# C0ldstudy/PointSecGuard

Measured on AMD Instinct MI355X. Metric: attacked rooms/sec (4096 pts, 40 PGD iters), higher is better.
Workload: dtype f32; 1 GPU; NB non-targeted PGD (eps=0.05, alpha=2/255, 40 iters) on PointNet++ SSG sem_seg, batch=8 rooms x 4096 pts x 9 ch per GPU (BASELINE configs[1]); steps_coalesced_per_launch_max=8, device_batch_rooms=64, launches_in_flight_per_gpu=3, weights=tests/golden/pn2_weights.npz (fitted fixture)

## Files before the change

pointsecguard_amd/csrc/psg_pn2.hip:

```cpp
#include <algorithm>
#include <cstdlib>
#include <cstring>
#include <vector>

#include "psg_common.h"
#include "psg_pn2_kernels.cuh"
#include "psg_chain.cuh"
#include "psg_pn2_geomgrad.cuh"

using namespace psg;

namespace {

constexpr int MAXL = PSG_PN2_MSG_NUM_LAYERS;
constexpr int NCLS = PSG_PN2_NUM_CLASSES;
const int kS[4] = {1024, 256, 64, 16};

static inline int diag_build_bits()
{
#ifdef PSG_DIAG_BUILD
    static const int bits = psg::env_int("PSG_DIAG", 0);
    return bits;
#else
    return 0;
// ... 91 lines not shown
    return arch_split(A, lvl) || (l0 && A.id == PSG_PN2_ARCH_SSG && lvl == 0);
}

bool arch_fp_split(const ArchDesc &A, int lvl)
{
    static const bool on = psg::env_int("PSG_PN2_FPSPLIT", 1) != 0, wave1 = psg::env_int("PSG_FP1_WAVE", 0) != 0;
    return on && lvl <= 2 && !(lvl == 0 && wave1);
}

bool arch_pack(const ArchDesc &A)
{
    static const bool on = psg::env_int("PSG_PN2_PACK", 1) != 0;
    return on && A.id == PSG_PN2_ARCH_SSG;
}

constexpr int kPackBwdBuilt = 1 << 0;
int pack_bwd_levels()
{
    static const int levels = [] {
        const char *v = psg::env_str("PSG_PN2_PACK_BWD");
        if (!v || !*v) return kPackBwdBuilt;
        if (*v == 'L' || *v == 'l') {
            int mask = 1 << 8;
            for (const char *c = v + 1; *c; ++c)
                if (*c >= '0' && *c <= '3') mask |= 1 << (*c - '0');
            return mask;
        }
        return atoi(v) != 0 ? kPackBwdBuilt : 0;
    }();
    return levels;
}
// ... 172 lines not shown
    EvScope prof(&ws->prof, tag, 0.0, st);
    hipLaunchKernelGGL(kern, grid, dim3(threads), lds, st, args);
    PSG_LAUNCH_CHECK_AT(site);
    return PSG_OK;
}

inline int layer_blocks(int k8, int mb) { return std::max(k8, mb * 4); }
inline int gsa_stride(const ArchDesc &A, int lvl)
{
    if (arch_split(A, lvl)) return A.cout[A.sc[lvl][0].l0];
    return lvl == 0 ? 12 : A.C[lvl];
}

#define PSG_CFG_KEY(P, NW, KS, MT) ((P) * 10000 + (NW) * 1000 + (KS) * 10 + (MT))

bool sa_pack_bwd_level(const psg_pn2_model *m, const psg_pn2_ws *ws, int lvl)
{
    const int levels = pack_bwd_levels();
    if (!ws->pk_cnt[lvl] || !((levels >> lvl) & 1)) return false;
    if (levels >> 8) return true;
    return lvl == 0 && !m->split_fwd[0] && !m->split[0] && m->split[1];
}

int run_sa_fwd(psg_pn2_model *m, psg_pn2_ws *ws, int lvl, int sc, int fwd, const float *x0, hipStream_t st)
{
    const ArchDesc &A = *m->arch;
    const ScaleDesc &d = A.sc[lvl][sc];
    const int B = ws->B, S = kS[lvl], Np = ws->Nl[lvl], D = A.C[lvl], KS = d.K, P = d.P, NW = d.NW;
    const PackedLayer *L = &m->L[d.l0];
    const size_t prob = (size_t)fwd * B;
    SaFwdArgs a;
    a.diag = diag_build_bits();
    a.xyz = lvl == 0 ? x0 : ws->xyz[lvl] + prob * Np * 3;
    a.xyz_stride = lvl == 0 ? 9 : 3;
    a.feat = lvl == 0 ? x0 : ws->act[lvl - 1];
    a.new_xyz = ws->xyz[lvl + 1] + prob * S * 3;
// ... 15 lines not shown
        return PSG_ERR_STATE;
    }
    const dim3 grid(S / (P / KS), B);
    const int tag = TAG_SA_FWD + lvl;
    a.pk_desc = nullptr; a.pk_tab_off = 0;
    const int blk = P * 8 + PSG_LDS_PAD;
    const bool pkm = sa_pack_bwd_level(m, ws, lvl);
    if (ws->pk_cnt[lvl] && KS == 32 && d.maxt_f == 1 && split == (lvl >= 1) && a.nb3 * (P / 32) == 2 * NW &&
        blocks * blk + 2 * P <= (P - 1) * a.C3 && (P * a.C3) % blk == 0) {
        a.pk_desc = ws->pk_desc[lvl] + prob * grid.x;
        a.pk_tab_off = blocks * blk;
        const int pblocks = P * a.C3 / blk;
        if (pkm) {
            switch (PSG_CFG_KEY(P, NW, KS, split ? 1 : 0)) {
            case PSG_CFG_KEY(128, 4, 32, 0): return launch_lds(ws, tag, PSG_SITE "#packed", (sa_fwd_packed_kernel<128, 4, false, true>), grid, 4 * 64, pblocks, blk, a, st);
            }
            set_error("run_sa_fwd level %d: PSG_PN2_PACK_BWD names a level without a packed-key forward kernel (P=%d NW=%d)", lvl, P, NW);
            return PSG_ERR_STATE;
        }
        switch (PSG_CFG_KEY(P, NW, KS, split ? 1 : 0)) {
        case PSG_CFG_KEY(128, 4, 32, 0): return launch_lds(ws, tag, PSG_SITE "#packed", (sa_fwd_packed_kernel<128, 4, false>), grid, 4 * 64, pblocks, blk, a, st);
        case PSG_CFG_KEY(64, 4, 32, 1): return launch_lds(ws, tag, PSG_SITE "#packed", (sa_fwd_packed_kernel<64, 4, true>), grid, 4 * 64, pblocks, blk, a, st);
        case PSG_CFG_KEY(32, 4, 32, 1): return launch_lds(ws, tag, PSG_SITE "#packed", (sa_fwd_packed_kernel<32, 4, true>), grid, 4 * 64, pblocks, blk, a, st);
        case PSG_CFG_KEY(32, 8, 32, 1): return launch_lds(ws, tag, PSG_SITE "#packed", (sa_fwd_packed_kernel<32, 8, true>), grid, 8 * 64, pblocks, blk, a, st);
        }
        a.pk_desc = nullptr; a.pk_tab_off = 0;
    }
    if (pkm) {
        set_error("run_sa_fwd level %d: the packed backward (PSG_PN2_PACK_BWD) needs the packed forward, which this configuration does not run", lvl);
        return PSG_ERR_STATE;
// ... 73 lines not shown
        a.nninv_off = ws->inv_off[3] + prob * (kS[3] + 1);
        a.nninv_ent = ws->inv_ent[3] + prob * ws->Nl[3] * 3;
        a.dint = ws->dint[3];
        a.n_fine = ws->Nl[3];
    }
    a.arg = ws->arg[lvl][sc];
    a.gidx = ws->gidx[lvl][sc] + prob * S * KS;
    a.l3t = bwd_layer(L[2], ws->mask[d.l0 + 1]);
    a.l2t = bwd_layer(L[1], ws->mask[d.l0]);
    a.l1t = bwd_layer(L[0], nullptr);
    a.D = D; a.Np = Np; a.S = S; a.C3 = C3;
    a.c_lo = c_lo; a.c_hi = c_hi;
    static const bool l1t_colour = psg::env_int("PSG_PN2_L1T_COLOUR", 1) != 0;
    a.w1c = nullptr; a.C1 = L[0].cout; a.w1c_off = 0;
    if (l1t_colour && a.cg_out == 4 && !a.split && P == 32 * NW && (a.C1 == 16 || a.C1 == 32)) a.w1c = m->w1feat[sc];
    static const bool poolt_sparse = psg::env_int("PSG_PN2_POOLT_SPARSE", 1) != 0;
    const int C2 = L[2].cin, NT = NW * 64;
    const int spv = poolt_sparse && L[2].wr && KS == 32 && P <= 64 && (P / KS) * C3 <= NT && C3 % 64 == 0 && !a.w1c &&
                    (C2 == 64 || C2 == 128 || C2 == 256) ? C2 / 64 : 0;
    const int l3_blocks = spv ? a.l3t.mb * 4 : layer_blocks(a.l3t.k8, a.l3t.mb);
    const int main_blocks = std::max(std::max(l3_blocks, layer_blocks(a.l2t.k8, a.l2t.mb)),
                                     a.split ? 0 : layer_blocks(a.l1t.k8, a.l1t.mb)) + PSG_LDS_SPARE;
    a.dsrc_blk = main_blocks;
    const int blk_floats = P * 8 + PSG_LDS_PAD;
    a.w1c_off = round_up((P / KS) * C3, 4);
    a.pos_off = a.w1c_off + (a.w1c ? round_up(3 * a.C1, 4) : 0);
    a.sp_off = round_up(a.pos_off + P, 4);
    a.w3r = spv ? L[2].wr : nullptr;
    const bool packed = sa_pack_bwd_level(m, ws, lvl);
    if (packed) {
        if (spv || a.split || !a.dout || a.nninv_off || a.ginv_off || ((a.ld | a.c_off) & 3) || (C3 & 7) ||
            PSG_CFG_KEY(P, NW, KS, d.maxt_b) != PSG_CFG_KEY(128, 4, 32, 1)) {
            set_error("run_sa_bwd level %d: PSG_PN2_PACK_BWD names a level without a packed backward kernel in this configuration", lvl);
            return PSG_ERR_STATE;
        }
    }
    const int staged = spv ? a.sp_off + 2 * NT + NW * 32 + P + 1 : a.pos_off + P + (packed ? P : 0);
    const int blocks = main_blocks + ceil_div(staged, blk_floats);
    if (std::max(std::max(a.l3t.mb, a.l2t.mb), a.split ? 0 : a.l1t.mb) * (P / 32) > d.maxt_b * NW) {
        set_error("run_sa_bwd level %d scale %d: more than %d tiles per wave in a layer", lvl, sc, d.maxt_b);
        return PSG_ERR_STATE;
    }
    const dim3 grid(S / (P / KS), B);
    const int tag = TAG_SA_BWD + lvl;
    if (packed) {
        const SaBwdPackedArgs pa{a, ws->pk_desc[lvl] + prob * grid.x};
        if (a.w1c) return launch_lds(ws, tag, PSG_SITE "#colour#bwd#packed", (sa_bwd_packed_kernel<128, 4, 1, 0>), grid, 4 * 64, blocks, Lds<128>::BLK, pa, st);
        return launch_lds(ws, tag, PSG_SITE "#bwd#packed", (sa_bwd_packed_kernel<128, 4, 1, 0>), grid, 4 * 64, blocks, Lds<128>::BLK, pa, st);
    }
#define PSG_SA_BWD_CASE(P_, NW_, KS_, MT_) \
    case PSG_CFG_KEY(P_, NW_, KS_, MT_): \
        if (a.w1c) return launch_lds(ws, tag, PSG_SITE "#colour", (sa_bwd_kernel<P_, NW_, MT_, KS_>), grid, NW_ * 64, blocks, Lds<P_>::BLK, a, st); \
        return launch_lds(ws, tag, PSG_SITE, (sa_bwd_kernel<P_, NW_, MT_, KS_>), grid, NW_ * 64, blocks, Lds<P_>::BLK, a, st)
    if (spv) {
        switch (PSG_CFG_KEY(P, NW, KS, d.maxt_b) * 8 + spv) {
        case PSG_CFG_KEY(64, 4, 32, 2) * 8 + 1: return launch_lds(ws, tag, PSG_SITE, (sa_bwd_sparse_kernel<64, 4, 2, 1>), grid, 4 * 64, blocks, Lds<64>::BLK, a, st);
        case PSG_CFG_KEY(32, 4, 32, 2) * 8 + 2: return launch_lds(ws, tag, PSG_SITE, (sa_bwd_sparse_kernel<32, 4, 2, 2>), grid, 4 * 64, blocks, Lds<32>::BLK, a, st);
        case PSG_CFG_KEY(32, 8, 32, 2) * 8 + 4: return launch_lds(ws, tag, PSG_SITE, (sa_bwd_sparse_kernel<32, 8, 2, 4>), grid, 8 * 64, blocks, Lds<32>::BLK, a, st);
        }
        set_error("run_sa_bwd: no sparse kernel for P=%d NW=%d MAXT=%d C2=%d", P, NW, d.maxt_b, C2);
        return PSG_ERR_STATE;
// ... 1304 lines not shown
```

pointsecguard_amd/csrc/psg_pn2_kernels.cuh:

```cuda
#pragma once
#include "psg_mlp.cuh"

#ifdef PSG_DIAG_BUILD
#define PSG_DIAGBIT(a, bit) ((a).diag & (bit))
#else
#define PSG_DIAGBIT(a, bit) 0
#endif

namespace psg {

struct SaFwdArgs {
    const float *xyz;
    const float *feat;
    const float *new_xyz;
    const int32_t *gidx;
    float *out;
    uint8_t *arg;
    FwdLayer l1, l2;
    const float4 *w3;
    const float *b3;
    int k8_3, nb3;
    int xyz_stride, D, Np, S, C3;
    int ld_out, c_out;
    const float *tfeat;
// ... 607 lines not shown
        const float4 z = *(const float4 *)(buf0 + L::off(c, j));
        const float4 w0 = *(const float4 *)(t + 4 * q), w1 = *(const float4 *)(t + KH + 4 * q), w2 = *(const float4 *)(t + 2 * KH + 4 * q);
        g0 = fmaf(z.x, w0.x, g0); g0 = fmaf(z.y, w0.y, g0); g0 = fmaf(z.z, w0.z, g0); g0 = fmaf(z.w, w0.w, g0);
        g1 = fmaf(z.x, w1.x, g1); g1 = fmaf(z.y, w1.y, g1); g1 = fmaf(z.z, w1.z, g1); g1 = fmaf(z.w, w1.w, g1);
        g2 = fmaf(z.x, w2.x, g2); g2 = fmaf(z.y, w2.y, g2); g2 = fmaf(z.z, w2.z, g2); g2 = fmaf(z.w, w2.w, g2);
    }
    const float o0 = __shfl_xor(g0, 32), o1 = __shfl_xor(g1, 32), o2 = __shfl_xor(g2, 32);
    if (h == 0 && pj >= 0) *(float4 *)(orow + (size_t)pj * 4) = make_float4(g0 + o0, g1 + o1, g2 + o2, 0.0f);
}

template <int SPV> struct SpVec;
template <> struct SpVec<1> { using T = float; };
template <> struct SpVec<2> { using T = float2; };
template <> struct SpVec<4> { using T = float4; };

template <int P, int NW, int MAXT, int SPV>
__device__ __forceinline__ void sa_pool_t_sparse(const SaBwdArgs &a, float *__restrict__ buf0, float *__restrict__ dsrc, int key,
                                                 size_t wg)
{
    using L = Lds<P>;
    using VT = typename SpVec<SPV>::T;
    constexpr int KS = 32, C2 = 64 * SPV, NT = NW * 64, PB = P / 32, U = 16;
    static_assert(P <= 64, "one scan lane per row");
    const int tid = threadIdx.x, lane = tid & 63, wave = tid >> 6;
    int2 *items = (int2 *)(dsrc + a.sp_off);
    int *tab = (int *)(items + NT);
    int *rs = tab + NW * KS;
    unsigned long long same = ~0ull;
#pragma unroll
    for (int bit = 0; bit < 6; ++bit) {
        const unsigned long long bb = __ballot((key >> bit) & 1);
        same &= ((key >> bit) & 1) ? bb : ~bb;
    }
    const int rank = __popcll(same & ((1ull << lane) - 1ull));
    if (key < KS && rank == 0) tab[wave * KS + key] = __popcll(same);
    __syncthreads();
    if (wave == 0) {
        const int cpg = a.C3 >> 6, g = lane / KS, k = lane & (KS - 1);
        int tot = 0;
        if (lane < P)
            for (int q = 0; q < cpg; ++q) tot += tab[(g * cpg + q) * KS + k];
        int inc = tot;
#pragma unroll
        for (int o = 1; o < 64; o <<= 1) {
            const int v = __shfl_up(inc, o);
            if (lane >= o) inc += v;
        }
        int run = inc - tot;
        if (lane < P) {
            rs[lane] = run;
            for (int q = 0; q < cpg; ++q) {
                int *t = tab + (g * cpg + q) * KS + k;
                const int c = *t;
                *t = run;
                run += c;
            }
        }
        if (lane == 63) rs[P] = inc;
    }
    __syncthreads();
    if (key < KS) {
        const int g = tid / a.C3, c = tid - g * a.C3;
        items[tab[wave * KS + key] + rank] = make_int2(((g * KS + key) << 16) | c, __float_as_int(dsrc[tid]));
    }
    const int ntask = (C2 / 32) * PB;
    unsigned msk[MAXT];
#pragma unroll
    for (int i = 0; i < MAXT; ++i) {
        const int task = wave + i * NW;
        msk[i] = 0xFFFFu;
        if (task < ntask && a.l3t.mask) msk[i] = a.l3t.mask[(wg * ntask + task) * 64 + lane];
    }
    __syncthreads();
    const int T = __builtin_amdgcn_readfirstlane(rs[P]);
    const int lo = wave * T / NW, hi = (wave + 1) * T / NW;
    const int rsl = lane < P ? rs[lane] : 0x7fffffff;
    const int r_lo = __popcll(__ballot(rsl < lo));
    const int r_hi = wave == NW - 1 ? P : __popcll(__ballot(rsl < hi));
    const int e_lo = __builtin_amdgcn_readfirstlane(rs[r_lo]), e_hi = __builtin_amdgcn_readfirstlane(rs[r_hi]);
    const float *wr = a.w3r + lane * SPV;
    float acc[SPV];
#pragma unroll
    for (int e = 0; e < SPV; ++e) acc[e] = 0.0f;
    int cur = r_lo;
    auto put = [&](int r) {
        float *o = buf0 + L::off(lane * SPV, r);
        if constexpr (SPV == 4) *(float4 *)o = make_float4(acc[0], acc[1], acc[2], acc[3]);
        else if constexpr (SPV == 2) *(float2 *)o = make_float2(acc[0], acc[1]);
        else *o = acc[0];
#pragma unroll
        for (int e = 0; e < SPV; ++e) acc[e] = 0.0f;
    };
    for (int w0 = e_lo; w0 < e_hi; w0 += 64) {
        const int n = min(64, e_hi - w0);
        const int2 mine = lane < n ? items[w0 + lane] : make_int2(0, 0);
        for (int q = 0; q < n; q += U) {
            VT w[U];
            int xs[U];
            float ds[U];
#pragma unroll
            for (int u = 0; u < U; ++u) {
                xs[u] = __builtin_amdgcn_readlane(mine.x, q + u);
                ds[u] = __int_as_float(__builtin_amdgcn_readlane(mine.y, q + u));
                if (q + u < n) w[u] = *(const VT *)(wr + (size_t)(xs[u] & 0xFFFF) * C2);
            }
#pragma unroll
            for (int u = 0; u < U; ++u) {
                if (q + u < n) {
                    const int row = xs[u] >> 16;
                    while (cur < row) put(cur++);
                    const float *wv = (const float *)&w[u];
#pragma unroll
                    for (int e = 0; e < SPV; ++e) acc[e] = fmaf(ds[u], wv[e], acc[e]);
                }
            }
        }
    }
    while (cur < r_hi) put(cur++);
    __syncthreads();
    const int j = lane & 31, h = lane >> 5;
#pragma unroll
    for (int i = 0; i < MAXT; ++i) {
        const int task = wave + i * NW;
        if (task < ntask) {
            const int mb = task / PB, pb = task - mb * PB;
            float *o = buf0 + (size_t)(mb * 4) * L::BLK + (pb * 32 + j) * 8 + 4 * h;
#pragma unroll
            for (int g = 0; g < 4; ++g) {
                float4 v = *(float4 *)(o + (size_t)g * L::BLK);
                v.x = __uint_as_float(__float_as_uint(v.x) & (unsigned)__builtin_amdgcn_sbfe((int)msk[i], 4 * g, 1));
                v.y = __uint_as_float(__float_as_uint(v.y) & (unsigned)__builtin_amdgcn_sbfe((int)msk[i], 4 * g + 1, 1));
                v.z = __uint_as_float(__float_as_uint(v.z) & (unsigned)__builtin_amdgcn_sbfe((int)msk[i], 4 * g + 2, 1));
                v.w = __uint_as_float(__float_as_uint(v.w) & (unsigned)__builtin_amdgcn_sbfe((int)msk[i], 4 * g + 3, 1));
                *(float4 *)(o + (size_t)g * L::BLK) = v;
            }
        }
    }
}

template <int P, int NW, int MAXT, int KS, int SPV, bool KEYED = false>
__device__ __forceinline__ void sa_bwd_body(const SaBwdArgs &a, int kbx = 0, int kb = 0, size_t kwg = 0)
{
    using L = Lds<P>;
    static_assert(KS == 32 || KS == 16, "groups of 32 or 16 samples");
    constexpr bool SPARSE = SPV > 0;
    static_assert(!SPARSE || KS == 32, "sparse max-pool transpose: groups of 32 samples");
    constexpr int G = P / KS, NT = NW * 64;
    extern __shared__ float lds[];
    float *buf0 = lds;
    const int tid = threadIdx.x;
    int bx, b;
    if constexpr (KEYED) { bx = kbx; b = kb; }
// ... 19 lines not shown
                const int pnt = t % P, blk = t / P;
                am_pre[i] = *(const uint2 *)(a.arg + ((size_t)b * a.S + s0 + pnt / KS) * a.C3 + blk * 8);
            }
        }
    }
    float *dsrc = lds + (size_t)a.dsrc_blk * L::BLK;
    if (SPARSE && tid < NW * KS) ((int *)(dsrc + a.sp_off) + 2 * NT)[tid] = 0;
    int32_t *s_pos = (int32_t *)(dsrc + a.pos_off);
    if (!a.w1c && tid < P) s_pos[tid] = a.gpos_out[(size_t)b * a.S * KS + (size_t)s0 * KS + tid];
    if (a.w1c && tid < 3 * a.C1) {
        const int kh = a.C1 >> 1, hh = tid / (3 * kh), r = (tid / kh) % 3, cc = tid % kh;
        dsrc[a.w1c_off + tid] = a.w1c[(hh * kh + cc) * a.D + a.c_lo + r];
    }
    for (int t = tid; t < G * a.C3; t += NT) {
        const int g = t / a.C3, c = t - g * a.C3;
        const int cc = a.c_off + c;
        float acc = a.dout ? a.dout[((size_t)b * a.S + s0 + g) * a.ld + cc] : 0.0f;
        if (a.nninv_off) {
            const int32_t *off = a.nninv_off + (size_t)b * (a.S + 1) + s0 + g;
            const int2 *ent = a.nninv_ent + (size_t)b * 3 * a.n_fine;
            const float *drows = a.dint + (size_t)b * a.n_fine * a.ld + cc;
            const int e1 = off[1];
            int e = off[0];
            for (; e + 4 <= e1; e += 4) {
                const int2 p0 = ent[e], p1 = ent[e + 1], p2 = ent[e + 2], p3 = ent[e + 3];
                const float v0 = drows[(size_t)p0.x * a.ld], v1 = drows[(size_t)p1.x * a.ld], v2 = drows[(size_t)p2.x * a.ld],
                            v3 = drows[(size_t)p3.x * a.ld];
                acc += __int_as_float(p0.y) * v0; acc += __int_as_float(p1.y) * v1;
                acc += __int_as_float(p2.y) * v2; acc += __int_as_float(p3.y) * v3;
            }
// ... 46 lines not shown
            v0.y = (int)((am.x >> 8) & 0xFF) == k ? d0.y : 0.f;
            v0.z = (int)((am.x >> 16) & 0xFF) == k ? d0.z : 0.f;
            v0.w = (int)(am.x >> 24) == k ? d0.w : 0.f;
            v1.x = (int)(am.y & 0xFF) == k ? d1.x : 0.f;
            v1.y = (int)((am.y >> 8) & 0xFF) == k ? d1.y : 0.f;
            v1.z = (int)((am.y >> 16) & 0xFF) == k ? d1.z : 0.f;
            v1.w = (int)(am.y >> 24) == k ? d1.w : 0.f;
            float *dst = buf0 + (size_t)blk * L::BLK + pnt * 8;
            *(float4 *)dst = v0;
            *(float4 *)(dst + 4) = v1;
        }
        __syncthreads();
        if (!PSG_DIAGBIT(a, 8)) layer_bwd<P, NW, MAXT>(a.l3t, buf0, wg);
    }
    if (!PSG_DIAGBIT(a, 16)) __syncthreads();
    if (!PSG_DIAGBIT(a, 8)) layer_bwd<P, NW, MAXT>(a.l2t, buf0, wg);
    if (!PSG_DIAGBIT(a, 16)) __syncthreads();
    if constexpr (P == 32 * NW) {
        if (a.w1c) {
            float *orowc = a.gsa_out + (size_t)b * a.S * KS * 4;
            const int32_t *posc = a.gpos_out + (size_t)b * a.S * KS + (size_t)s0 * KS;
            if (a.C1 == 32) sa_l1t_colour<P, NW, 32>(a, buf0, dsrc + a.w1c_off, posc, orowc);
            else sa_l1t_colour<P, NW, 16>(a, buf0, dsrc + a.w1c_off, posc, orowc);
            return;
        }
    }
    if (!a.split) {
        if (!PSG_DIAGBIT(a, 8)) layer_bwd<P, NW, MAXT>(a.l1t, buf0, wg);
        __syncthreads();
    }
    if (PSG_DIAGBIT(a, 32)) return;
// ... 53 lines not shown
            apply_bits(c, m);
            acc[i] = c;
        }
    }
    __syncthreads();
#pragma unroll
    for (int i = 0; i < MAXT; ++i) {
        const int task = first + i * NW;
        if (task < ntask) {
            const int mb = task / nblk, pb = task - mb * nblk;
            store_tile<P>(buf, mb, pb * 32 + j, h, acc[i]);
        }
    }
}

template <int P, int NW, int MAXT, int SPV>
__global__ __launch_bounds__(NW * 64) void sa_bwd_packed_kernel(SaBwdPackedArgs pa)
{
    const SaBwdArgs &a = pa.a;
    using L = Lds<P>;
    static_assert(SPV == 0 && MAXT == 1 && P == 32 * NW, "built: the dense level, one tile per wave");
    constexpr int PB = P / 32, NT = NW * 64, KS = 32;
    extern __shared__ float lds[];
    float *buf0 = lds;
    const int tid = threadIdx.x, wave = tid >> 6;
    int bx, b;
    xcd_tile(bx, b);
    const size_t wg = (size_t)b * gridDim.x + bx;
    const int4 desc = pa.pk_desc[wg];
    const int ng = desc.x >> 16, sA = desc.x & 0xFFFF;
    if (ng == 0) return;
    int nrows = 0, rg_g = 0, rg_st = 0;
    for (int i = 0; i < ng; ++i) {
        if (tid >= nrows) { rg_g = i; rg_st = nrows; }
        nrows += sa_pack_cnt(desc, i);
    }
    if (ng == PB && (sA & (PB - 1)) == 0 && nrows == P) {
        sa_bwd_body<P, NW, MAXT, KS, 0, true>(a, sA / PB, b, wg);
        return;
    }
    const int nblk = (nrows + 31) >> 5, nact = nblk * 32;
    float *dsrc = lds + (size_t)a.dsrc_blk * L::BLK;
    int32_t *s_pos = (int32_t *)(dsrc + a.pos_off);
    int *s_row = s_pos + P;
    if (tid < P) {
        int om = -1, pj = -1;
        if (tid < nrows) {
            const int k = tid - rg_st;
            om = (rg_g << 5) | k;
            pj = a.gpos_out[(size_t)b * a.S * KS + (size_t)(sA + rg_g) * KS + k];
        }
        s_row[tid] = om;
        s_pos[tid] = pj;
    }
    if (a.w1c && tid < 3 * a.C1) {
        const int kh = a.C1 >> 1, hh = tid / (3 * kh), r = (tid / kh) % 3, cc = tid % kh;
        dsrc[a.w1c_off + tid] = a.w1c[(hh * kh + cc) * a.D + a.c_lo + r];
    }
    __syncthreads();
    {
        const float *drows = a.dout + (size_t)b * a.S * a.ld + a.c_off;
        const uint8_t *arows = a.arg + (size_t)b * a.S * a.C3;
        const int nq = nblk * (a.C3 >> 3);
        const int rcp = (65536 + nblk - 1) / nblk;
#pragma unroll
        for (int i = 0; i < 4; ++i) {
            const int q = (tid >> 5) + i * (NT / 32);
            if (q < nq) {
                const int blk = (q * rcp) >> 16, pb = q - blk * nblk, j = pb * 32 + (tid & 31);
                const int om = s_row[j];
                float4 v0 = make_float4(0.f, 0.f, 0.f, 0.f), v1 = v0;
                if (om >= 0) {
                    const int s = sA + (om >> 5), k = om & 31;
                    const uint2 am = *(const uint2 *)(arows + (size_t)s * a.C3 + blk * 8);
                    const float *dp = drows + (size_t)s * a.ld + blk * 8;
                    const float4 d0 = *(const float4 *)dp, d1 = *(const float4 *)(dp + 4);
                    v0.x = (int)(am.x & 0xFF) == k ? d0.x : 0.f;
                    v0.y = (int)((am.x >> 8) & 0xFF) == k ? d0.y : 0.f;
                    v0.z = (int)((am.x >> 16) & 0xFF) == k ? d0.z : 0.f;
                    v0.w = (int)(am.x >> 24) == k ? d0.w : 0.f;
                    v1.x = (int)(am.y & 0xFF) == k ? d1.x : 0.f;
                    v1.y = (int)((am.y >> 8) & 0xFF) == k ? d1.y : 0.f;
                    v1.z = (int)((am.y >> 16) & 0xFF) == k ? d1.z : 0.f;
                    v1.w = (int)(am.y >> 24) == k ? d1.w : 0.f;
                }
                float *dst = buf0 + (size_t)blk * L::BLK + j * 8;
                *(float4 *)dst = v0;
                *(float4 *)(dst + 4) = v1;
            }
        }
    }
    __syncthreads();
    sa_layer_bwd_packed<P, NW, MAXT>(a.l3t, buf0, nblk, wg);
    __syncthreads();
    sa_layer_bwd_packed<P, NW, MAXT>(a.l2t, buf0, nblk, wg);
    __syncthreads();
    if (a.w1c) {
        if (wave < nblk) {
            float *orowc = a.gsa_out + (size_t)b * a.S * KS * 4;
            if (a.C1 == 32) sa_l1t_colour<P, NW, 32>(a, buf0, dsrc + a.w1c_off, s_pos, orowc);
            else sa_l1t_colour<P, NW, 16>(a, buf0, dsrc + a.w1c_off, s_pos, orowc);
        }
        return;
    }
    if (!a.split) {
        sa_layer_bwd_packed<P, NW, MAXT>(a.l1t, buf0, nblk, wg);
        __syncthreads();
    }
    const int nc = a.c_hi - a.c_lo;
    const int32_t *pos = s_pos;
    float *orow = a.gsa_out + (size_t)b * a.S * KS * a.cg_out;
    if (a.cg_out == 4) {
        for (int j = tid; j < nact; j += NT) {
            const float4 v = make_float4(buf0[L::off(a.c_lo, j)], buf0[L::off(a.c_lo + 1, j)], buf0[L::off(a.c_lo + 2, j)], 0.0f);
            if (pos[j] >= 0) *(float4 *)(orow + (size_t)pos[j] * 4) = v;
        }
        return;
    }
    if (((nc | a.c_lo | a.cg_out) & 3) == 0) {
        constexpr int RG = NT / 32;
        const int ql = tid & 31, rg = tid >> 5;
        for (int j = rg; j < nact; j += RG) {
// ... 613 lines not shown
```

Measured before the change: 957.3 rooms/s.

## Extend packed-row backward to sparse-pool SA levels 1-3

Enables the packed (compacted valid-row) backward path by default for SA level 1 as well as level 0, and adds packed forward/backward kernel instantiations for the split sparse-pool configurations at levels 1-3. A new packed variant of the sparse max-pool transpose scatters gradients straight into the compacted rows, iterating over groups and applying the ReLU mask tile once at the end. The goal is to skip work on padded or duplicate neighbour rows in the deeper levels. It adds extra LDS staging for group starts, a per-group loop with more barriers, and more kernel variants.

```diff
diff --git a/pointsecguard_amd/csrc/psg_pn2.hip b/pointsecguard_amd/csrc/psg_pn2.hip
--- a/pointsecguard_amd/csrc/psg_pn2.hip
+++ b/pointsecguard_amd/csrc/psg_pn2.hip
@@ -129,7 +129,7 @@
     return on && A.id == PSG_PN2_ARCH_SSG;
 }
 
-constexpr int kPackBwdBuilt = 1 << 0;
+constexpr int kPackBwdBuilt = (1 << 0) | (1 << 1);
 int pack_bwd_levels()
 {
     static const int levels = [] {
@@ -332,12 +332,22 @@
 
 #define PSG_CFG_KEY(P, NW, KS, MT) ((P) * 10000 + (NW) * 1000 + (KS) * 10 + (MT))
 
+int sa_sparse_spv(const ScaleDesc &d, const PackedLayer *L, bool w1c)
+{
+    static const bool poolt_sparse = psg::env_int("PSG_PN2_POOLT_SPARSE", 1) != 0;
+    const int C3 = L[2].cout, C2 = L[2].cin, NT = d.NW * 64;
+    return poolt_sparse && L[2].wr && d.K == 32 && d.P <= 64 && (d.P / d.K) * C3 <= NT && C3 % 64 == 0 && !w1c &&
+           (C2 == 64 || C2 == 128 || C2 == 256) ? C2 / 64 : 0;
+}
+
 bool sa_pack_bwd_level(const psg_pn2_model *m, const psg_pn2_ws *ws, int lvl)
 {
     const int levels = pack_bwd_levels();
     if (!ws->pk_cnt[lvl] || !((levels >> lvl) & 1)) return false;
     if (levels >> 8) return true;
-    return lvl == 0 && !m->split_fwd[0] && !m->split[0] && m->split[1];
+    if (lvl == 0) return !m->split_fwd[0] && !m->split[0] && m->split[1];
+    return m->split_fwd[lvl] && m->split[lvl] && (lvl == 3 || m->split[lvl + 1]) &&
+           sa_sparse_spv(m->arch->sc[lvl][0], &m->L[m->arch->sc[lvl][0].l0], false) > 0;
 }
 
 int run_sa_fwd(psg_pn2_model *m, psg_pn2_ws *ws, int lvl, int sc, int fwd, const float *x0, hipStream_t st)
@@ -383,6 +393,9 @@
         if (pkm) {
             switch (PSG_CFG_KEY(P, NW, KS, split ? 1 : 0)) {
             case PSG_CFG_KEY(128, 4, 32, 0): return launch_lds(ws, tag, PSG_SITE "#packed", (sa_fwd_packed_kernel<128, 4, false, true>), grid, 4 * 64, pblocks, blk, a, st);
+            case PSG_CFG_KEY(64, 4, 32, 1): return launch_lds(ws, tag, PSG_SITE "#packed", (sa_fwd_packed_kernel<64, 4, true, true>), grid, 4 * 64, pblocks, blk, a, st);
+            case PSG_CFG_KEY(32, 4, 32, 1): return launch_lds(ws, tag, PSG_SITE "#packed", (sa_fwd_packed_kernel<32, 4, true, true>), grid, 4 * 64, pblocks, blk, a, st);
+            case PSG_CFG_KEY(32, 8, 32, 1): return launch_lds(ws, tag, PSG_SITE "#packed", (sa_fwd_packed_kernel<32, 8, true, true>), grid, 8 * 64, pblocks, blk, a, st);
             }
             set_error("run_sa_fwd level %d: PSG_PN2_PACK_BWD names a level without a packed-key forward kernel (P=%d NW=%d)", lvl, P, NW);
             return PSG_ERR_STATE;
@@ -486,10 +499,8 @@
     static const bool l1t_colour = psg::env_int("PSG_PN2_L1T_COLOUR", 1) != 0;
     a.w1c = nullptr; a.C1 = L[0].cout; a.w1c_off = 0;
     if (l1t_colour && a.cg_out == 4 && !a.split && P == 32 * NW && (a.C1 == 16 || a.C1 == 32)) a.w1c = m->w1feat[sc];
-    static const bool poolt_sparse = psg::env_int("PSG_PN2_POOLT_SPARSE", 1) != 0;
     const int C2 = L[2].cin, NT = NW * 64;
-    const int spv = poolt_sparse && L[2].wr && KS == 32 && P <= 64 && (P / KS) * C3 <= NT && C3 % 64 == 0 && !a.w1c &&
-                    (C2 == 64 || C2 == 128 || C2 == 256) ? C2 / 64 : 0;
+    const int spv = sa_sparse_spv(d, L, a.w1c != nullptr);
     const int l3_blocks = spv ? a.l3t.mb * 4 : layer_blocks(a.l3t.k8, a.l3t.mb);
     const int main_blocks = std::max(std::max(l3_blocks, layer_blocks(a.l2t.k8, a.l2t.mb)),
                                      a.split ? 0 : layer_blocks(a.l1t.k8, a.l1t.mb)) + PSG_LDS_SPARE;
@@ -501,13 +512,18 @@
     a.w3r = spv ? L[2].wr : nullptr;
     const bool packed = sa_pack_bwd_level(m, ws, lvl);
     if (packed) {
-        if (spv || a.split || !a.dout || a.nninv_off || a.ginv_off || ((a.ld | a.c_off) & 3) || (C3 & 7) ||
-            PSG_CFG_KEY(P, NW, KS, d.maxt_b) != PSG_CFG_KEY(128, 4, 32, 1)) {
+        const bool dense0 = !spv && !a.split && a.dout && !a.nninv_off && !a.ginv_off && !((a.ld | a.c_off) & 3) && !(C3 & 7) &&
+                            PSG_CFG_KEY(P, NW, KS, d.maxt_b) == PSG_CFG_KEY(128, 4, 32, 1);
+        const bool sparse = spv && a.split && m->split_fwd[lvl] && !a.ginv_off && (a.dout != nullptr) != (a.nninv_off != nullptr) &&
+                            (P / KS) * C3 == NT && std::max(a.l3t.mb, a.l2t.mb) * (P / 32) <= NW &&
+                            (PSG_CFG_KEY(P, NW, KS, spv) == PSG_CFG_KEY(64, 4, 32, 1) || PSG_CFG_KEY(P, NW, KS, spv) == PSG_CFG_KEY(32, 4, 32, 2) ||
+                             PSG_CFG_KEY(P, NW, KS, spv) == PSG_CFG_KEY(32, 8, 32, 4));
+        if (!dense0 && !sparse) {
             set_error("run_sa_bwd level %d: PSG_PN2_PACK_BWD names a level without a packed backward kernel in this configuration", lvl);
             return PSG_ERR_STATE;
         }
     }
-    const int staged = spv ? a.sp_off + 2 * NT + NW * 32 + P + 1 : a.pos_off + P + (packed ? P : 0);
+    const int staged = spv ? a.sp_off + 2 * NT + NW * 32 + P + 1 + (packed ? SA_PACK_GCAP + 1 : 0) : a.pos_off + P + (packed ? P : 0);
     const int blocks = main_blocks + ceil_div(staged, blk_floats);
     if (std::max(std::max(a.l3t.mb, a.l2t.mb), a.split ? 0 : a.l1t.mb) * (P / 32) > d.maxt_b * NW) {
         set_error("run_sa_bwd level %d scale %d: more than %d tiles per wave in a layer", lvl, sc, d.maxt_b);
@@ -517,6 +533,11 @@
     const int tag = TAG_SA_BWD + lvl;
     if (packed) {
         const SaBwdPackedArgs pa{a, ws->pk_desc[lvl] + prob * grid.x};
+        switch (spv) {
+        case 1: return launch_lds(ws, tag, PSG_SITE "#sa2#bwd#packed", (sa_bwd_packed_kernel<64, 4, 1, 1>), grid, 4 * 64, blocks, Lds<64>::BLK, pa, st);
+        case 2: return launch_lds(ws, tag, PSG_SITE "#sa3#bwd#packed", (sa_bwd_packed_kernel<32, 4, 1, 2>), grid, 4 * 64, blocks, Lds<32>::BLK, pa, st);
+        case 4: return launch_lds(ws, tag, PSG_SITE "#sa4#bwd#packed", (sa_bwd_packed_kernel<32, 8, 1, 4>), grid, 8 * 64, blocks, Lds<32>::BLK, pa, st);
+        }
         if (a.w1c) return launch_lds(ws, tag, PSG_SITE "#colour#bwd#packed", (sa_bwd_packed_kernel<128, 4, 1, 0>), grid, 4 * 64, blocks, Lds<128>::BLK, pa, st);
         return launch_lds(ws, tag, PSG_SITE "#bwd#packed", (sa_bwd_packed_kernel<128, 4, 1, 0>), grid, 4 * 64, blocks, Lds<128>::BLK, pa, st);
     }
diff --git a/pointsecguard_amd/csrc/psg_pn2_kernels.cuh b/pointsecguard_amd/csrc/psg_pn2_kernels.cuh
--- a/pointsecguard_amd/csrc/psg_pn2_kernels.cuh
+++ b/pointsecguard_amd/csrc/psg_pn2_kernels.cuh
@@ -645,9 +645,25 @@
 template <> struct SpVec<2> { using T = float2; };
 template <> struct SpVec<4> { using T = float4; };
 
-template <int P, int NW, int MAXT, int SPV>
+template <int P>
+__device__ __forceinline__ void sa_mask_tile(float *__restrict__ buf0, int mb, int pb, int j, int h, unsigned m)
+{
+    using L = Lds<P>;
+    float *o = buf0 + (size_t)(mb * 4) * L::BLK + (pb * 32 + j) * 8 + 4 * h;
+#pragma unroll
+    for (int g = 0; g < 4; ++g) {
+        float4 v = *(float4 *)(o + (size_t)g * L::BLK);
+        v.x = __uint_as_float(__float_as_uint(v.x) & (unsigned)__builtin_amdgcn_sbfe((int)m, 4 * g, 1));
+        v.y = __uint_as_float(__float_as_uint(v.y) & (unsigned)__builtin_amdgcn_sbfe((int)m, 4 * g + 1, 1));
+        v.z = __uint_as_float(__float_as_uint(v.z) & (unsigned)__builtin_amdgcn_sbfe((int)m, 4 * g + 2, 1));
+        v.w = __uint_as_float(__float_as_uint(v.w) & (unsigned)__builtin_amdgcn_sbfe((int)m, 4 * g + 3, 1));
+        *(float4 *)(o + (size_t)g * L::BLK) = v;
+    }
+}
+
+template <int P, int NW, int MAXT, int SPV, bool PACKED = false>
 __device__ __forceinline__ void sa_pool_t_sparse(const SaBwdArgs &a, float *__restrict__ buf0, float *__restrict__ dsrc, int key,
-                                                 size_t wg)
+                                                 size_t wg, const int *__restrict__ gst = nullptr, float dval = 0.0f)
 {
     using L = Lds<P>;
     using VT = typename SpVec<SPV>::T;
@@ -657,116 +673,158 @@
     int2 *items = (int2 *)(dsrc + a.sp_off);
     int *tab = (int *)(items + NT);
     int *rs = tab + NW * KS;
-    unsigned long long same = ~0ull;
-#pragma unroll
-    for (int bit = 0; bit < 6; ++bit) {
-        const unsigned long long bb = __ballot((key >> bit) & 1);
-        same &= ((key >> bit) & 1) ? bb : ~bb;
-    }
-    const int rank = __popcll(same & ((1ull << lane) - 1ull));
-    if (key < KS && rank == 0) tab[wave * KS + key] = __popcll(same);
-    __syncthreads();
-    if (wave == 0) {
-        const int cpg = a.C3 >> 6, g = lane / KS, k = lane & (KS - 1);
-        int tot = 0;
-        if (lane < P)
-            for (int q = 0; q < cpg; ++q) tot += tab[(g * cpg + q) * KS + k];
-        int inc = tot;
-#pragma unroll
-        for (int o = 1; o < 64; o <<= 1) {
-            const int v = __shfl_up(inc, o);
-            if (lane >= o) inc += v;
-        }
-        int run = inc - tot;
-        if (lane < P) {
-            rs[lane] = run;
-            for (int q = 0; q < cpg; ++q) {
-                int *t = tab + (g * cpg + q) * KS + k;
-                const int c = *t;
-                *t = run;
-                run += c;
-            }
-        }
-        if (lane == 63) rs[P] = inc;
-    }
-    __syncthreads();
-    if (key < KS) {
-        const int g = tid / a.C3, c = tid - g * a.C3;
-        items[tab[wave * KS + key] + rank] = make_int2(((g * KS + key) << 16) | c, __float_as_int(dsrc[tid]));
+    if (!PSG_DIAGBIT(a, 1024)) {
+        unsigned long long same = ~0ull;
+#pragma unroll
+        for (int bit = 0; bit < 6; ++bit) {
+            const unsigned long long bb = __ballot((key >> bit) & 1);
+            same &= ((key >> bit) & 1) ? bb : ~bb;
+        }
+        const int rank = __popcll(same & ((1ull << lane) - 1ull));
+        if (key < KS && rank == 0) tab[wave * KS + key] = __popcll(same);
+        __syncthreads();
+        if (wave == 0) {
+            const int cpg = a.C3 >> 6, g = lane / KS, k = lane & (KS - 1);
+            int tot = 0;
+            if (lane < P)
+                for (int q = 0; q < cpg; ++q) tot += tab[(g * cpg + q) * KS + k];
+            int inc = tot;
+#pragma unroll
+            for (int o = 1; o < 64; o <<= 1) {
+                const int v = __shfl_up(inc, o);
+                if (lane >= o) inc += v;
+            }
+            int run = inc - tot;
+            if (lane < P) {
+                rs[lane] = run;
+                for (int q = 0; q < cpg; ++q) {
+                    int *t = tab + (g * cpg + q) * KS + k;
+                    const int c = *t;
+                    *t = run;
+                    run += c;
+                }
+            }
+            if (lane == 63) rs[P] = inc;
+        }
+        __syncthreads();
+        if (key < KS) {
+            const int g = tid / a.C3, c = tid - g * a.C3;
+            items[tab[wave * KS + key] + rank] = make_int2(((g * KS + key) << 16) | c, __float_as_int(PACKED ? dval : dsrc[tid]));
+        }
     }
     const int ntask = (C2 / 32) * PB;
     unsigned msk[MAXT];
-#pragma unroll
-    for (int i = 0; i < MAXT; ++i) {
-        const int task = wave + i * NW;
-        msk[i] = 0xFFFFu;
-        if (task < ntask && a.l3t.mask) msk[i] = a.l3t.mask[(wg * ntask + task) * 64 + lane];
-    }
-    __syncthreads();
-    const int T = __builtin_amdgcn_readfirstlane(rs[P]);
-    const int lo = wave * T / NW, hi = (wave + 1) * T / NW;
-    const int rsl = lane < P ? rs[lane] : 0x7fffffff;
-    const int r_lo = __popcll(__ballot(rsl < lo));
-    const int r_hi = wave == NW - 1 ? P : __popcll(__ballot(rsl < hi));
-    const int e_lo = __builtin_amdgcn_readfirstlane(rs[r_lo]), e_hi = __builtin_amdgcn_readfirstlane(rs[r_hi]);
-    const float *wr = a.w3r + lane * SPV;
-    float acc[SPV];
-#pragma unroll
-    for (int e = 0; e < SPV; ++e) acc[e] = 0.0f;
-    int cur = r_lo;
-    auto put = [&](int r) {
-        float *o = buf0 + L::off(lane * SPV, r);
-        if constexpr (SPV == 4) *(float4 *)o = make_float4(acc[0], acc[1], acc[2], acc[3]);
-        else if constexpr (SPV == 2) *(float2 *)o = make_float2(acc[0], acc[1]);
-        else *o = acc[0];
+    if constexpr (!PACKED) {
+#pragma unroll
+        for (int i = 0; i < MAXT; ++i) {
+            const int task = wave + i * NW;
+            msk[i] = 0xFFFFu;
+            if (task < ntask && a.l3t.mask && !PSG_DIAGBIT(a, 2048)) msk[i] = a.l3t.mask[(wg * ntask + task) * 64 + lane];
+        }
+    }
+    __syncthreads();
+    if (!PSG_DIAGBIT(a, 128 | 1024)) {
+        const int T = __builtin_amdgcn_readfirstlane(rs[P]);
+        const int lo = wave * T / NW, hi = (wave + 1) * T / NW;
+        const int rsl = lane < P ? rs[lane] : 0x7fffffff;
+        const int r_lo = __popcll(__ballot(rsl < lo));
+        const int r_hi = wave == NW - 1 ? P : __popcll(__ballot(rsl < hi));
+        const int e_lo = __builtin_amdgcn_readfirstlane(rs[r_lo]), e_hi = __builtin_amdgcn_readfirstlane(rs[r_hi]);
+        const float *wr = a.w3r + lane * SPV;
+        float acc[SPV];
 #pragma unroll
         for (int e = 0; e < SPV; ++e) acc[e] = 0.0f;
-    };
-    for (int w0 = e_lo; w0 < e_hi; w0 += 64) {
-        const int n = min(64, e_hi - w0);
-        const int2 mine = lane < n ? items[w0 + lane] : make_int2(0, 0);
-        for (int q = 0; q < n; q += U) {
-            VT w[U];
-            int xs[U];
-            float ds[U];
-#pragma unroll
-            for (int u = 0; u < U; ++u) {
-                xs[u] = __builtin_amdgcn_readlane(mine.x, q + u);
-                ds[u] = __int_as_float(__builtin_amdgcn_readlane(mine.y, q + u));
-                if (q + u < n) w[u] = *(const VT *)(wr + (size_t)(xs[u] & 0xFFFF) * C2);
-            }
-#pragma unroll
-            for (int u = 0; u < U; ++u) {
-                if (q + u < n) {
-                    const int row = xs[u] >> 16;
-                    while (cur < row) put(cur++);
-                    const float *wv = (const float *)&w[u];
-#pragma unroll
-                    for (int e = 0; e < SPV; ++e) acc[e] = fmaf(ds[u], wv[e], acc[e]);
+        int cur = r_lo;
+        int dstv = -1;
+        if constexpr (PACKED) {
+            if (lane < P) {
+                const int st = gst[lane >> 5], k = lane & 31;
+                if (k < gst[(lane >> 5) + 1] - st) dstv = st + k;
+            }
+            if (lane < KS) tab[wave * KS + lane] = 0;
+        }
+        auto put = [&](int r) {
+            if constexpr (PACKED) {
+                r = __builtin_amdgcn_readlane(dstv, r);
+                if (r < 0) return;
+            }
+            float *o = buf0 + L::off(lane * SPV, r);
+            if constexpr (SPV == 4) *(float4 *)o = make_float4(acc[0], acc[1], acc[2], acc[3]);
+            else if constexpr (SPV == 2) *(float2 *)o = make_float2(acc[0], acc[1]);
+            else *o = acc[0];
+#pragma unroll
+            for (int e = 0; e < SPV; ++e) acc[e] = 0.0f;
+        };
+        for (int w0 = e_lo; w0 < e_hi; w0 += 64) {
+            const int n = min(64, e_hi - w0);
+            const int2 mine = lane < n ? items[w0 + lane] : make_int2(0, 0);
+            for (int q = 0; q < n; q += U) {
+                VT w[U];
+                int xs[U];
+                float ds[U];
+#pragma unroll
+                for (int u = 0; u < U; ++u) {
+                    xs[u] = __builtin_amdgcn_readlane(mine.x, q + u);
+                    ds[u] = __int_as_float(__builtin_amdgcn_readlane(mine.y, q + u));
+                    if (q + u < n) w[u] = *(const VT *)(wr + (size_t)(xs[u] & 0xFFFF) * C2);
                 }
-            }
-        }
-    }
-    while (cur < r_hi) put(cur++);
-    __syncthreads();
-    const int j = lane & 31, h = lane >> 5;
-#pragma unroll
-    for (int i = 0; i < MAXT; ++i) {
-        const int task = wave + i * NW;
-        if (task < ntask) {
-            const int mb = task / PB, pb = task - mb * PB;
-            float *o = buf0 + (size_t)(mb * 4) * L::BLK + (pb * 32 + j) * 8 + 4 * h;
-#pragma unroll
-            for (int g = 0; g < 4; ++g) {
-                float4 v = *(float4 *)(o + (size_t)g * L::BLK);
-                v.x = __uint_as_float(__float_as_uint(v.x) & (unsigned)__builtin_amdgcn_sbfe((int)msk[i], 4 * g, 1));
-                v.y = __uint_as_float(__float_as_uint(v.y) & (unsigned)__builtin_amdgcn_sbfe((int)msk[i], 4 * g + 1, 1));
-                v.z = __uint_as_float(__float_as_uint(v.z) & (unsigned)__builtin_amdgcn_sbfe((int)msk[i], 4 * g + 2, 1));
-                v.w = __uint_as_float(__float_as_uint(v.w) & (unsigned)__builtin_amdgcn_sbfe((int)msk[i], 4 * g + 3, 1));
-                *(float4 *)(o + (size_t)g * L::BLK) = v;
-            }
-        }
-    }
+#pragma unroll
+                for (int u = 0; u < U; ++u) {
+                    if (q + u < n) {
+                        const int row = xs[u] >> 16;
+                        while (cur < row) put(cur++);
+                        const float *wv = (const float *)&w[u];
+#pragma unroll
+                        for (int e = 0; e < SPV; ++e) acc[e] = fmaf(ds[u], wv[e], acc[e]);
+                    }
+                }
+            }
+        }
+        while (cur < r_hi) put(cur++);
+    }
+    if constexpr (!PACKED) {
+        __syncthreads();
+        const int j = lane & 31, h = lane >> 5;
+#pragma unroll
+        for (int i = 0; i < MAXT; ++i) {
+            const int task = wave + i * NW;
+            if (task < ntask && !PSG_DIAGBIT(a, 2048)) {
+                const int mb = task / PB, pb = task - mb * PB;
+                float *o = buf0 + (size_t)(mb * 4) * L::BLK + (pb * 32 + j) * 8 + 4 * h;
+#pragma unroll
+                for (int g = 0; g < 4; ++g) {
+                    float4 v = *(float4 *)(o + (size_t)g * L::BLK);
+                    v.x = __uint_as_float(__float_as_uint(v.x) & (unsigned)__builtin_amdgcn_sbfe((int)msk[i], 4 * g, 1));
+                    v.y = __uint_as_float(__float_as_uint(v.y) & (unsigned)__builtin_amdgcn_sbfe((int)msk[i], 4 * g + 1, 1));
+                    v.z = __uint_as_float(__float_as_uint(v.z) & (unsigned)__builtin_amdgcn_sbfe((int)msk[i], 4 * g + 2, 1));
+                    v.w = __uint_as_float(__float_as_uint(v.w) & (unsigned)__builtin_amdgcn_sbfe((int)msk[i], 4 * g + 3, 1));
+                    *(float4 *)(o + (size_t)g * L::BLK) = v;
+                }
+            }
+        }
+    }
+}
+
+__device__ __forceinline__ float sa_nninv_grad(const SaBwdArgs &a, int b, int s, int c)
+{
+    const int32_t *off = a.nninv_off + (size_t)b * (a.S + 1) + s;
+    const int2 *ent = a.nninv_ent + (size_t)b * 3 * a.n_fine;
+    const float *drows = a.dint + (size_t)b * a.n_fine * a.ld + a.c_off + c;
+    const int e1 = off[1];
+    int e = off[0];
+    float acc = 0.0f;
+    for (; e + 4 <= e1; e += 4) {
+        const int2 p0 = ent[e], p1 = ent[e + 1], p2 = ent[e + 2], p3 = ent[e + 3];
+        const float v0 = drows[(size_t)p0.x * a.ld], v1 = drows[(size_t)p1.x * a.ld], v2 = drows[(size_t)p2.x * a.ld],
+                    v3 = drows[(size_t)p3.x * a.ld];
+        acc += __int_as_float(p0.y) * v0; acc += __int_as_float(p1.y) * v1;
+        acc += __int_as_float(p2.y) * v2; acc += __int_as_float(p3.y) * v3;
+    }
+    for (; e < e1; ++e) {
+        const int2 pe = ent[e];
+        acc += __int_as_float(pe.y) * drows[(size_t)pe.x * a.ld];
+    }
+    return acc;
 }
 
 template <int P, int NW, int MAXT, int KS, int SPV, bool KEYED = false>
@@ -816,6 +874,7 @@
     }
     for (int t = tid; t < G * a.C3; t += NT) {
         const int g = t / a.C3, c = t - g * a.C3;
+        if (PSG_DIAGBIT(a, 4096)) { dsrc[t] = 0.0f; continue; }
         const int cc = a.c_off + c;
         float acc = a.dout ? a.dout[((size_t)b * a.S + s0 + g) * a.ld + cc] : 0.0f;
         if (a.nninv_off) {
@@ -892,7 +951,7 @@
         if (!PSG_DIAGBIT(a, 8)) layer_bwd<P, NW, MAXT>(a.l3t, buf0, wg);
     }
     if (!PSG_DIAGBIT(a, 16)) __syncthreads();
-    if (!PSG_DIAGBIT(a, 8)) layer_bwd<P, NW, MAXT>(a.l2t, buf0, wg);
+    if (!PSG_DIAGBIT(a, 8 | 2048)) layer_bwd<P, NW, MAXT>(a.l2t, buf0, wg);
     if (!PSG_DIAGBIT(a, 16)) __syncthreads();
     if constexpr (P == 32 * NW) {
         if (a.w1c) {
@@ -976,12 +1035,60 @@
     }
 }
 
+template <int P, int NW, int SPV>
+__device__ __forceinline__ void sa_bwd_packed_sparse(const SaBwdArgs &a, float *__restrict__ buf0, float *__restrict__ dsrc,
+                                                     const int4 &desc, int b, size_t wg, int nrows)
+{
+    using L = Lds<P>;
+    constexpr int G = P / 32, PB = P / 32, NT = NW * 64, KS = 32, C2 = 64 * SPV, GCAP = SA_PACK_GCAP;
+    const int tid = threadIdx.x, lane = tid & 63, wave = tid >> 6;
+    const int ng = desc.x >> 16, sA = desc.x & 0xFFFF;
+    const int nblk = (nrows + 31) >> 5;
+    int *tab = (int *)(dsrc + a.sp_off) + 2 * NT;
+    int *gstart = tab + NW * KS + P + 1;
+    {
+        int st = 0;
+        for (int i = 0; i < ng; ++i) {
+            if (tid == i) gstart[i] = st;
+            st += sa_pack_cnt(desc, i);
+        }
+        if (tid >= ng && tid <= GCAP) gstart[tid] = nrows;
+    }
+    for (int t = tid; t < (nblk * 32 - nrows) * (C2 / 4); t += NT) {
+        const int r = nrows + t / (C2 / 4), q = t % (C2 / 4);
+        *(float4 *)(buf0 + L::off(4 * q, r)) = make_float4(0.f, 0.f, 0.f, 0.f);
+    }
+    const int mb = wave / nblk, pb = wave - mb * nblk;
+    const bool mtile = wave < (C2 / 32) * nblk;
+    unsigned msk = 0xFFFFu;
+    if (mtile && a.l3t.mask) msk = a.l3t.mask[((wg * (C2 / 32) + mb) * PB + pb) * 64 + lane];
+    const int gl = tid / a.C3, c = tid - gl * a.C3;
+    const uint8_t *arow = a.arg + ((size_t)b * a.S + sA) * a.C3 + c;
+    const bool plain = !a.nninv_off;
+    const float *drow = plain ? a.dout + ((size_t)b * a.S + sA) * a.ld + a.c_off + c : nullptr;
+    if (tid < NW * KS) tab[tid] = 0;
+    __syncthreads();
+    for (int g0 = 0; g0 < ng; g0 += G) {
+        int key = KS;
+        float dv = 0.0f;
+        if (g0 + gl < ng) {
+            const int v = arow[(size_t)(g0 + gl) * a.C3];
+            key = v == 255 ? KS : v;
+            dv = plain ? drow[(size_t)(g0 + gl) * a.ld] : sa_nninv_grad(a, b, sA + g0 + gl, c);
+        }
+        sa_pool_t_sparse<P, NW, 1, SPV, true>(a, buf0, dsrc, key, wg, gstart + g0, dv);
+    }
+    __syncthreads();
+    if (mtile) sa_mask_tile<P>(buf0, mb, pb, lane & 31, lane >> 5, msk);
+    __syncthreads();
+}
+
 template <int P, int NW, int MAXT, int SPV>
 __global__ __launch_bounds__(NW * 64) void sa_bwd_packed_kernel(SaBwdPackedArgs pa)
 {
     const SaBwdArgs &a = pa.a;
     using L = Lds<P>;
-    static_assert(SPV == 0 && MAXT == 1 && P == 32 * NW, "built: the dense level, one tile per wave");
+    static_assert(MAXT == 1 && (SPV > 0 ? P <= 64 : P == 32 * NW), "one tile per wave in every layer");
     constexpr int PB = P / 32, NT = NW * 64, KS = 32;
     extern __shared__ float lds[];
     float *buf0 = lds;
@@ -998,76 +1105,83 @@
         nrows += sa_pack_cnt(desc, i);
     }
     if (ng == PB && (sA & (PB - 1)) == 0 && nrows == P) {
-        sa_bwd_body<P, NW, MAXT, KS, 0, true>(a, sA / PB, b, wg);
+        sa_bwd_body<P, NW, (SPV > 0 ? 2 : MAXT), KS, SPV, true>(a, sA / PB, b, wg);
         return;
     }
     const int nblk = (nrows + 31) >> 5, nact = nblk * 32;
     float *dsrc = lds + (size_t)a.dsrc_blk * L::BLK;
     int32_t *s_pos = (int32_t *)(dsrc + a.pos_off);
-    int *s_row = s_pos + P;
-    if (tid < P) {
-        int om = -1, pj = -1;
-        if (tid < nrows) {
-            const int k = tid - rg_st;
-            om = (rg_g << 5) | k;
-            pj = a.gpos_out[(size_t)b * a.S * KS + (size_t)(sA + rg_g) * KS + k];
-        }
-        s_row[tid] = om;
-        s_pos[tid] = pj;
-    }
-    if (a.w1c && tid < 3 * a.C1) {
-        const int kh = a.C1 >> 1, hh = tid / (3 * kh), r = (tid / kh) % 3, cc = tid % kh;
-        dsrc[a.w1c_off + tid] = a.w1c[(hh * kh + cc) * a.D + a.c_lo + r];
-    }
-    __syncthreads();
-    {
-        const float *drows = a.dout + (size_t)b * a.S * a.ld + a.c_off;
-        const uint8_t *arows = a.arg + (size_t)b * a.S * a.C3;
-        const int nq = nblk * (a.C3 >> 3);
-        const int rcp = (65536 + nblk - 1) / nblk;
-#pragma unroll
-        for (int i = 0; i < 4; ++i) {
-            const int q = (tid >> 5) + i * (NT / 32);
-            if (q < nq) {
-                const int blk = (q * rcp) >> 16, pb = q - blk * nblk, j = pb * 32 + (tid & 31);
-                const int om = s_row[j];
-                float4 v0 = make_float4(0.f, 0.f, 0.f, 0.f), v1 = v0;
-                if (om >= 0) {
-                    const int s = sA + (om >> 5), k = om & 31;
-                    const uint2 am = *(const uint2 *)(arows + (size_t)s * a.C3 + blk * 8);
-                    const float *dp = drows + (size_t)s * a.ld + blk * 8;
-                    const float4 d0 = *(const float4 *)dp, d1 = *(const float4 *)(dp + 4);
-                    v0.x = (int)(am.x & 0xFF) == k ? d0.x : 0.f;
-                    v0.y = (int)((am.x >> 8) & 0xFF) == k ? d0.y : 0.f;
-                    v0.z = (int)((am.x >> 16) & 0xFF) == k ? d0.z : 0.f;
-                    v0.w = (int)(am.x >> 24) == k ? d0.w : 0.f;
-                    v1.x = (int)(am.y & 0xFF) == k ? d1.x : 0.f;
-                    v1.y = (int)((am.y >> 8) & 0xFF) == k ? d1.y : 0.f;
-                    v1.z = (int)((am.y >> 16) & 0xFF) == k ? d1.z : 0.f;
-                    v1.w = (int)(am.y >> 24) == k ? d1.w : 0.f;
+    if constexpr (SPV > 0) {
+        if (tid < P) s_pos[tid] = tid < nrows ? a.gpos_out[(size_t)b * a.S * KS + (size_t)(sA + rg_g) * KS + tid - rg_st] : -1;
+        sa_bwd_packed_sparse<P, NW, SPV>(a, buf0, dsrc, desc, b, wg, nrows);
+    } else {
+        int *s_row = s_pos + P;
+        if (tid < P) {
+            int om = -1, pj = -1;
+            if (tid < nrows) {
+                const int k = tid - rg_st;
+                om = (rg_g << 5) | k;
+                pj = a.gpos_out[(size_t)b * a.S * KS + (size_t)(sA + rg_g) * KS + k];
+            }
+            s_row[tid] = om;
+            s_pos[tid] = pj;
+        }
+        if (a.w1c && tid < 3 * a.C1) {
+            const int kh = a.C1 >> 1, hh = tid / (3 * kh), r = (tid / kh) % 3, cc = tid % kh;
+            dsrc[a.w1c_off + tid] = a.w1c[(hh * kh + cc) * a.D + a.c_lo + r];
+        }
+        __syncthreads();
+        {
+            const float *drows = a.dout + (size_t)b * a.S * a.ld + a.c_off;
+            const uint8_t *arows = a.arg + (size_t)b * a.S * a.C3;
+            const int nq = nblk * (a.C3 >> 3);
+            const int rcp = (65536 + nblk - 1) / nblk;
+#pragma unroll
+            for (int i = 0; i < 4; ++i) {
+                const int q = (tid >> 5) + i * (NT / 32);
+                if (q < nq) {
+                    const int blk = (q * rcp) >> 16, pb = q - blk * nblk, j = pb * 32 + (tid & 31);
+                    const int om = s_row[j];
+                    float4 v0 = make_float4(0.f, 0.f, 0.f, 0.f), v1 = v0;
+                    if (om >= 0) {
+                        const int s = sA + (om >> 5), k = om & 31;
+                        const uint2 am = *(const uint2 *)(arows + (size_t)s * a.C3 + blk * 8);
+                        const float *dp = drows + (size_t)s * a.ld + blk * 8;
+                        const float4 d0 = *(const float4 *)dp, d1 = *(const float4 *)(dp + 4);
+                        v0.x = (int)(am.x & 0xFF) == k ? d0.x : 0.f;
+                        v0.y = (int)((am.x >> 8) & 0xFF) == k ? d0.y : 0.f;
+                        v0.z = (int)((am.x >> 16) & 0xFF) == k ? d0.z : 0.f;
+                        v0.w = (int)(am.x >> 24) == k ? d0.w : 0.f;
+                        v1.x = (int)(am.y & 0xFF) == k ? d1.x : 0.f;
+                        v1.y = (int)((am.y >> 8) & 0xFF) == k ? d1.y : 0.f;
+                        v1.z = (int)((am.y >> 16) & 0xFF) == k ? d1.z : 0.f;
+                        v1.w = (int)(am.y >> 24) == k ? d1.w : 0.f;
+                    }
+                    float *dst = buf0 + (size_t)blk * L::BLK + j * 8;
+                    *(float4 *)dst = v0;
+                    *(float4 *)(dst + 4) = v1;
                 }
-                float *dst = buf0 + (size_t)blk * L::BLK + j * 8;
-                *(float4 *)dst = v0;
-                *(float4 *)(dst + 4) = v1;
-            }
-        }
-    }
-    __syncthreads();
-    sa_layer_bwd_packed<P, NW, MAXT>(a.l3t, buf0, nblk, wg);
-    __syncthreads();
+            }
+        }
+        __syncthreads();
+        sa_layer_bwd_packed<P, NW, MAXT>(a.l3t, buf0, nblk, wg);
+        __syncthreads();
+    }
     sa_layer_bwd_packed<P, NW, MAXT>(a.l2t, buf0, nblk, wg);
     __syncthreads();
-    if (a.w1c) {
-        if (wave < nblk) {
-            float *orowc = a.gsa_out + (size_t)b * a.S * KS * 4;
-            if (a.C1 == 32) sa_l1t_colour<P, NW, 32>(a, buf0, dsrc + a.w1c_off, s_pos, orowc);
-            else sa_l1t_colour<P, NW, 16>(a, buf0, dsrc + a.w1c_off, s_pos, orowc);
-        }
-        return;
-    }
-    if (!a.split) {
-        sa_layer_bwd_packed<P, NW, MAXT>(a.l1t, buf0, nblk, wg);
-        __syncthreads();
+    if constexpr (SPV == 0) {
+        if (a.w1c) {
+            if (wave < nblk) {
+                float *orowc = a.gsa_out + (size_t)b * a.S * KS * 4;
+                if (a.C1 == 32) sa_l1t_colour<P, NW, 32>(a, buf0, dsrc + a.w1c_off, s_pos, orowc);
+                else sa_l1t_colour<P, NW, 16>(a, buf0, dsrc + a.w1c_off, s_pos, orowc);
+            }
+            return;
+        }
+        if (!a.split) {
+            sa_layer_bwd_packed<P, NW, MAXT>(a.l1t, buf0, nblk, wg);
+            __syncthreads();
+        }
     }
     const int nc = a.c_hi - a.c_lo;
     const int32_t *pos = s_pos;
```

After: 968.7 rooms/s (median of 6 runs). +1.2%, better.
